# zwu88/TANTE

Measured on AMD Instinct MI355X. Metric: rollout frames/sec (fwd), TANTE on 256x256 Active Matter, higher is better.
Workload: dtype bf16

## Files before the change

### tante_amd/_lib.py

```python
import ctypes as C
import os

HERE = os.path.dirname(os.path.abspath(__file__))
LIB_PATH = os.environ.get("TANTE_LIB") or os.path.join(HERE, "lib", "libtante_hip.so")

F32, BF16 = 0, 1
ACT_NONE, ACT_GELU_ERF, ACT_GELU_TANH, ACT_RELU = 0, 1, 2, 3
A_LINEAR, A_PATCH_NHWC, A_PATCH_NCHW = 0, 1, 2
E_LINEAR, E_FILM, E_DECONV_NHWC, E_DECONV_NCHW = 0, 1, 2, 3
W_LINEAR, W_CONV_NHWC, W_DECONV_NHWC, W_DECONV_NCHW = 0, 1, 2, 3
W_LINEAR_T, W_CONV_NHWC_T, W_DECONV_NHWC_T, W_DECONV_NCHW_T = 4, 5, 6, 7

c_i32, c_i64, c_f32, c_vp = C.c_int32, C.c_int64, C.c_float, C.c_void_p


class PackGeom(C.Structure):
    _fields_ = [("n_pad", c_i32), ("k_pad", c_i32), ("nt", c_i32), ("cb", c_i32), ("bytes", c_i64)]


class Gemm(C.Structure):
    _fields_ = [
        ("a", c_vp), ("a_dtype", c_i32), ("a_mode", c_i32), ("M", c_i32), ("K", c_i32),
        ("a_s1", c_i64), ("a_s0", c_i64), ("a_off", c_i64), ("a_n0", c_i32),
        ("Hin", c_i32), ("Win", c_i32), ("Cin", c_i32), ("P", c_i32), ("ln", c_i32), ("ln_eps", c_f32),
# ... 144 lines not shown
                                   c_i64, c_i64, c_vp, c_vp], c_i32),
    "tante_cross_attention": ([c_vp, c_vp, c_vp, c_vp, c_i32, c_i64, c_i32, c_i32, c_i32, c_i32, c_i64, c_i64, c_i64, c_vp], c_i32),
    "tante_cvit_chain512": ([c_vp, c_vp, c_i64, c_vp, c_vp, c_vp, c_vp, c_f32, c_f32, c_f32, c_vp, c_vp, c_i32, c_i64, c_i32, c_vp, c_vp], c_i32),
    "tante_cvit_chain512_qkv": ([c_vp, c_vp, c_i64, c_vp, c_vp, c_f32, c_f32, c_i64, c_vp, c_vp, c_vp], c_i32),
    "tante_cross_attention_q": ([c_vp, c_vp, c_vp, c_vp, c_i32, c_i64, c_i32, c_i32, c_i32, c_i32, c_i64, c_i64, c_i64, c_i64, c_vp], c_i32),
    "tante_cross_attention_bwd": ([c_vp] * 9 + [c_i32, c_i64, c_i32, c_i32, c_i32, c_i32, c_i64, c_i64, c_i64, c_i64, c_vp], c_i32),
    "tante_layernorm_affine_bwd": ([c_vp, c_i32, c_vp, c_i32, c_vp, c_i64, c_i32, c_f32, c_vp, c_vp, c_vp, c_vp], c_i32),
    "tante_grid_embed_bwd": ([c_vp] * 5 + [c_i64, c_i32, c_i32, c_f32, c_vp, c_vp, c_vp, c_vp], c_i32),
    "tante_grid_embed": ([c_vp, c_vp, c_vp, c_i64, c_i32, c_i32, c_f32, c_vp, c_vp], c_i32),
    "tante_fourier_embed": ([c_vp, c_vp, c_i64, c_i32, c_vp, c_vp], c_i32),
    "tante_metric_sums": ([c_vp, c_i64, c_i64, c_i64, c_i64, c_vp, c_i32, c_i32, c_i64, c_i32, c_vp, c_vp], c_i32),
    "tante_mse_grad": ([c_vp, c_i64, c_i64, c_i64, c_i64, c_vp, c_i32, c_i32, c_i64, c_i32, c_f32, c_vp, c_vp], c_i32),
    "tante_sumsq": ([c_vp, c_i64, c_vp, c_vp], c_i32),
    "tante_adamw_step": ([c_vp, c_vp, c_vp, c_vp, c_i64, c_vp, c_f32, c_f32, c_f32, c_f32, c_f32, c_f32, c_i32, c_f32, c_vp], c_i32),
    "tante_layernorm_fwd": ([c_vp, c_i64, c_i32, c_f32, c_vp, c_i32, c_vp, c_vp], c_i32),
    "tante_layernorm_bwd": ([c_vp, c_i32, c_vp, c_vp, c_vp, c_i64, c_i32, c_vp, c_vp], c_i32),
    "tante_act_fwd": ([c_vp, c_i32, c_vp, c_i32, c_i64, c_i32, c_vp], c_i32),
    "tante_act_bwd": ([c_vp, c_i32, c_vp, c_i32, c_vp, c_i32, c_i64, c_i32, c_vp], c_i32),
    "tante_colsum": ([c_vp, c_i32, c_i64, c_i32, c_i64, c_vp, c_i32, c_vp], c_i32),
    "tante_film_pos_fwd": ([c_vp, c_vp, c_vp, c_vp, c_i64, c_i32, c_i32, c_i64, c_vp, c_vp], c_i32),
    "tante_pos_embed_tmajor": ([c_vp, c_vp, c_vp, c_i64, c_i32, c_i64, c_i32, c_vp, c_vp], c_i32),
    "tante_film_pos_bwd": ([c_vp, c_vp, c_vp, c_i64, c_i64, c_i32, c_i32, c_vp, c_vp, c_vp, c_vp, c_vp], c_i32),
    "tante_taylor_bwd": ([c_vp, c_i64, C.POINTER(c_vp), c_i32, C.c_double, c_i32, c_vp, c_i64, c_i32, c_i64, c_i64, c_vp], c_i32),
    "tante_attention_bwd": ([c_vp, c_vp, c_vp, c_i32, c_i32, c_i32, C.POINTER(Seq), c_i32, c_f32, C.c_uint64, c_vp], c_i32),
    "tante_attention_dropout": ([c_vp, c_vp, c_i32, c_i32, c_i32, C.POINTER(Seq), c_i32, c_f32, C.c_uint64, c_vp], c_i32),
    "tante_dropout_add": ([c_vp, c_i32, c_vp, c_f32, C.c_uint64, c_i64, c_vp, c_vp], c_i32),
    "tante_dropout_bwd": ([c_vp, c_f32, C.c_uint64, c_i64, c_vp, c_i32, c_vp], c_i32),
    "tante_axis_mlp_bwd": ([c_vp, c_vp, c_i64, c_i32, c_i64, c_vp, c_vp, c_vp, c_vp, c_vp, c_vp, c_vp], c_i32),
    "tante_fold_fwd": ([c_vp, c_vp, c_vp, c_vp, c_i32, c_i32, c_vp, c_vp, c_vp], c_i32),
    "tante_fold_bwd": ([c_vp, c_vp, c_vp, c_vp, c_vp, c_i32, c_i32, c_vp, c_vp, c_vp, c_vp, c_vp], c_i32),
    "tante_fold_bwd_clear": ([c_vp, c_vp, c_vp, c_vp, c_vp, c_i32, c_i32, c_vp, c_vp, c_vp, c_vp, c_vp], c_i32),
    "tante_fold_bwd_multi": ([c_vp, c_i32, c_i32, c_vp], c_i32),
    "tante_fold_fwd_multi": ([c_vp, c_i32, c_vp], c_i32),
    "tante_axis_mlp_film_supported": ([c_i64, c_i32, c_i32, c_i64, c_i32], c_i32),
    "tante_axis_mlp_film": ([c_vp, c_vp, c_vp, c_vp, c_vp, c_i64, c_i32, c_i32, c_i64, c_i32, c_vp, c_vp, c_vp, c_vp, c_vp], c_i32),
    "tante_film_pos_fwd_frames": ([c_vp, c_vp, c_vp, c_vp, c_i64, c_i32, c_i64, c_i32, c_vp, c_vp], c_i32),
    "tante_film_pos_bwd_frames": ([c_vp, c_vp, c_vp, c_i64, c_i64, c_i32, c_i32, c_vp, c_vp, c_vp, c_vp, c_vp], c_i32),
    "tante_film_pos_bwd_frames_acc": ([c_vp, c_vp, c_vp, c_i64, c_i64, c_i32, c_i32, c_vp, c_i32, c_vp, c_vp, c_vp, c_i32, c_vp], c_i32),
    "tante_film_table_bwd": ([c_vp, c_i32, c_i32] + [c_vp] * 6 + [c_vp, c_vp] + [c_vp] * 8 + [c_i32, c_vp], c_i32),
    "tante_pack_block_train_multi": ([c_vp, c_i32, c_i32, c_i32, c_vp], c_i32),
    "tante_pack_block_tail_bwd_multi": ([c_vp, c_i32, c_i32, c_i32, c_vp], c_i32),
    "tante_axis_mlp_bwd_fused_supported": ([c_i32, c_i64], c_i32),
    "tante_axis_mlp_bwd_fused": ([c_vp, c_vp, c_i64, c_i32, c_i64, c_vp, c_vp, c_vp, c_vp, c_vp, c_vp, c_vp, c_vp, c_vp], c_i32),
    "tante_axis_mlp_bwd_fused_ws": ([c_vp, c_vp, c_i64, c_i32, c_i64, c_vp, c_vp, c_vp, c_vp, c_vp, c_vp, c_vp, c_vp, c_vp, c_i64, c_vp], c_i32),
    "tante_axis_wgrad": ([c_vp, c_vp, c_i64, c_i32, c_i64, c_vp, c_vp, c_i32, c_vp], c_i32),
    "tante_axis_wgrad_workspace_bytes": ([], c_i64),
    "tante_set_seed_mix": ([c_vp], c_i32),
    "tante_axis_wgrad_ws": ([c_vp, c_vp, c_i64, c_i32, c_i64, c_vp, c_vp, c_i32, c_vp, c_i64, c_vp], c_i32),
    "tante_wgrad": ([C.POINTER(RowMat), C.POINTER(RowMat), c_i64, c_i32, c_i32, c_vp, c_vp, c_i32, c_i32, c_i32, c_i32, c_i32, c_i32, c_vp], c_i32),
    "tante_wgrad_ws": ([C.POINTER(RowMat), C.POINTER(RowMat), c_i64, c_i32, c_i32, c_vp, c_vp, c_i32, c_i32, c_i32, c_i32, c_i32, c_i32, c_vp, c_i64, c_vp], c_i32),
    "tante_wgrad_multi_ws": ([c_vp, c_vp, c_i32, c_i64, c_i32, c_i32, c_vp, c_vp, c_i32, c_i32, c_i32, c_i32, c_i32, c_i32, c_vp, c_i64, c_vp], c_i32),
    "tante_wgrad_multi": ([c_vp, c_vp, c_i32, c_i64, c_i32, c_i32, c_vp, c_vp, c_i32, c_i32, c_i32, c_i32, c_i32, c_i32, c_vp], c_i32),
    "tante_clip_value": ([c_vp, c_i64, c_f32, c_vp], c_i32),
    "tante_rt_reduce_bwd": ([c_vp, c_i32, c_i32, c_vp, c_vp], c_i32),
    "tante_last_error": ([], C.c_char_p),
    "tante_abi_version": ([], c_i32),
    "tante_set_option": ([C.c_char_p, c_i32], c_i32),
    "tante_nan_to_num": ([c_vp, c_vp, c_i64, c_vp], c_i32),
    "tante_head_fused_multi": ([c_i32, c_vp, c_vp, c_vp, c_i32, c_i64, c_i64, c_i64, c_i32, c_i32, c_i32, c_i32, c_i32, c_vp, c_i64, c_vp, c_i64,
                               c_vp], c_i32),
    "tante_head_fused_multi_streams": ([c_i32, c_vp, c_vp, c_vp, c_i32, c_i64, c_i64, c_i64, c_i32, c_i32, c_i32, c_i32, c_i32, c_vp, c_i64, c_vp, c_i64,
                               c_vp], c_i32),
    "tante_spectral_bf16out_supported": ([c_i64, c_i32, c_i32, c_i32, c_i32, c_i32, c_i32], c_i32),
    "tante_spectral_layer_bf16out": ([c_vp, c_i64, c_i32, c_i32, c_i32, c_vp, c_vp, c_i32, c_i32, c_i32, c_i32, c_vp, c_vp, c_i32, c_i32, c_vp, c_vp,
                                     c_i64, c_vp], c_i32),
    "tante_get_option": ([C.c_char_p, c_i32], c_i32),
    "tante_attention_masked": ([c_vp, c_vp, c_i32, c_i32, c_i32, c_i32, c_i32, c_i32, c_vp, c_i64, c_vp, c_vp], c_i32),
    "tante_attention_masked_bwd": ([c_vp, c_vp, c_vp, c_i32, c_i32, c_i32, c_i32, c_i32, c_i32, c_vp, c_i64, c_vp, c_vp, c_vp], c_i32),
    "tante_attention_flash_stats_floats": ([c_i32, C.POINTER(Seq)], c_i64),
    "tante_attention_flash_supported": ([c_i32, c_i32, c_i32, c_i32], c_i32),
    "tante_attention_flash": ([c_vp, c_vp, c_vp, c_i32, c_i32, c_i32, C.POINTER(Seq), c_i32, c_f32, C.c_uint64, c_vp], c_i32),
    "tante_attention_flash_bwd": ([c_vp, c_vp, c_vp, c_vp, c_vp, c_i32, c_i32, c_i32, C.POINTER(Seq), c_i32, c_f32, C.c_uint64, c_vp], c_i32),
    "tante_attention_flash_masked": ([c_vp, c_vp, c_vp, c_i32, c_i32, c_i32, c_i32, c_i32, c_i32, c_vp, c_i64, c_vp, c_f32, C.c_uint64, c_vp], c_i32),
    "tante_attention_flash_masked_bwd": ([c_vp, c_vp, c_vp, c_vp, c_vp, c_i32, c_i32, c_i32, c_i32, c_i32, c_i32, c_vp, c_i64, c_vp, c_f32, C.c_uint64, c_vp], c_i32),
    "tante_head_enc_supported": ([c_i32, c_i32], c_i32),
    "tante_head_enc_stream_bytes": ([c_i32], c_i64),
    "tante_head_enc_ws_bytes": ([c_i64], c_i64),
    "tante_pack_head_enc": ([c_vp] * 6 + [c_i32, c_i32, c_vp, c_vp], c_i32),
    "tante_head_enc_fused": ([c_i32, c_vp, c_vp, c_vp, c_i32, c_i64, c_i64, c_i64, c_i32, c_i32, c_i32, c_i32, c_i32, c_vp, c_i64, c_vp, c_i64,
                             c_vp, c_vp, c_vp, c_i64, c_vp], c_i32),
}

LIB_OPTIONS = ("TANTE_ATTN_BWD_HG", "TANTE_ATTN_BWD_NO_SPLIT", "TANTE_ATTN_BWD_VALU", "TANTE_ATTN_FWD_VALU", "TANTE_AXIS_BWD_SMALL_WGS",
               "TANTE_AXIS_BWD_WGS", "TANTE_AXIS_CT", "TANTE_AXIS_FILM", "TANTE_AXIS_GENERIC", "TANTE_AXIS_MFMA", "TANTE_AXIS_NT", "TANTE_AXIS_WGRAD_WGS",
               "TANTE_BLOCK_KERNEL", "TANTE_COLSUM_ROWS", "TANTE_CVIT_CHAIN_TOKENS", "TANTE_ENC23_SPLIT", "TANTE_FILM_BWD_ROWS",
               "TANTE_FS_GROUPS", "TANTE_FS_HALF", "TANTE_FS_SKEW", "TANTE_FS_WAVES", "TANTE_GEMM_NO_LITE", "TANTE_GEMM_SMALLM", "TANTE_GEMM_WGS", "TANTE_HEAD_WAVES",
               "TANTE_IM2COL_TILED", "TANTE_RESIZE_TILED", "TANTE_SPECTRAL_BF16OUT", "TANTE_SPECTRAL_DFT", "TANTE_SPECTRAL_X3", "TANTE_WGRAD_DEEP",
               "TANTE_WGRAD_JOBS", "TANTE_WGRAD_JOBS_WGS", "TANTE_WGRAD_NO_SLAB", "TANTE_WGRAD_NO_TR", "TANTE_WGRAD_REDUCE_NY",
               "TANTE_WGRAD_RG", "TANTE_WGRAD_SLAB_WGS", "TANTE_WGRAD_TR_WGS", "TANTE_WGRAD_WGS", "TANTE_XATTN_GPW", "TANTE_XATTN_VALU",)


_lib = None
ABI_VERSION = 14


def lib():
    global _lib
    if _lib is None:
        if not os.path.exists(LIB_PATH):
            raise RuntimeError(
                f"{LIB_PATH} is missing: build it with `python -m tante_amd.build` "
                "(or __graft_entry__.build()).  tante_amd has no CPU / eager fallback.")
        L = C.CDLL(LIB_PATH)
        for name, (argtypes, restype) in SIGNATURES.items():
            fn = getattr(L, name)
            fn.argtypes = argtypes
            fn.restype = restype
        got = int(L.tante_abi_version())
        if got != ABI_VERSION:
            raise RuntimeError(f"{LIB_PATH}: library ABI {got}, this binding expects {ABI_VERSION} -- a stale build (or a stale variant under "
                               "TANTE_LIB); rebuild with `python -m tante_amd.build`")
        _lib = L
        import warnings
        for k in LIB_OPTIONS:
            v = os.environ.get(k)
            if v is None:
                continue
            try:
                rc = L.tante_set_option(k.encode(), int(v))
            except ValueError:
                warnings.warn(f"{k}={v!r}: library options are integers; ignored")
                continue
            if rc != 0:
                warnings.warn(f"{k}={v}: tante_set_option refused it ({L.tante_last_error().decode(errors='replace')})")
    return _lib


def set_option(name: str, value: int) -> None:
    check(lib().tante_set_option(name.encode(), int(value)), "tante_set_option")


def get_option(name: str, default: int = 0) -> int:
    return int(lib().tante_get_option(name.encode(), int(default)))


def check(rc: int, what: str = ""):
    if rc != 0:
        msg = lib().tante_last_error().decode(errors="replace")
        raise RuntimeError(f"libtante_hip {what} failed (rc={rc}): {msg}")
```

### tante_amd/csrc/pointwise.hip

```cpp
#include "common.hip.h"
#include <stdlib.h>
#include <string.h>
#include <mutex>
#include <algorithm>

int tante_axis_mlp_mfma_supported(int64_t outer, int n, int64_t inner, const void* x, const void* w1, const void* w2);
int tante_axis_mlp_mfma(float* x, int64_t outer, int n, int64_t inner, const float* w1, const float* b1, const float* w2, const float* b2, hipStream_t s);

namespace {

template <int N>
__global__ __launch_bounds__(256) void axis_mlp_kernel(float* __restrict__ x, long outer, int n, long inner,
                                                       const float* __restrict__ w1, const float* __restrict__ b1,
                                                       const float* __restrict__ w2, const float* __restrict__ b2) {
  __shared__ __attribute__((aligned(16))) float w1s[N * N];
  __shared__ __attribute__((aligned(16))) float w2ts[N * N];
  __shared__ __attribute__((aligned(16))) float b1s[N];
  __shared__ __attribute__((aligned(16))) float b2s[N];
  for (int idx = threadIdx.x; idx < N * N; idx += 256) {
    const int j = idx / N, a = idx % N;
    const bool in = (j < n) && (a < n);
    w1s[idx] = in ? w1[j * n + a] : 0.0f;
    w2ts[idx] = in ? w2[a * n + j] : 0.0f;
  }
// ... 333 lines not shown
    const int tokn = i >> 2, q = i & 3, h = tokn / nW, w = tokn - h * nW;
    f32x4 v = *(const f32x4*)(lsrc + (long)tokn * C + q * 4);
    if (S.src) {
      const f32x4 a = *(const f32x4*)(fa + q * 4), b = *(const f32x4*)(fb + q * 4), sv = *(const f32x4*)(S.se + (long)tokn * C + c0 + q * 4);
      v = v * a + b + sv;
    }
    float2* d = (float2*)(plane + h * rs + w * AXWS + q * 4);
    d[0] = make_float2(v[0], v[1]);
    d[1] = make_float2(v[2], v[3]);
  }
  __syncthreads();
  if (!(dbg & 2)) axis_phase<BF16, MT>(plane, wst, wh1, bh1, wh2, bh2, nH, nW, rs, AXWS, tid);
  if (!(dbg & 4) && !(dbg & 1)) {
    axis_phase<BF16, MT>(plane, wst, ww1, bw1, ww2, bw2, nW, nH, AXWS, rs, tid, gx, (long)C, (long)nW * C);
    return;
  }
  if (!(dbg & 4)) axis_phase<BF16, MT>(plane, wst, ww1, bw1, ww2, bw2, nW, nH, AXWS, rs, tid);
  if (!(dbg & 1))
  for (int i = tid; i < nH * nW * 4; i += AXT) {
    const int tokn = i >> 2, q = i & 3, h = tokn / nW, w = tokn - h * nW;
    const float2* sp = (const float2*)(plane + h * rs + w * AXWS + q * 4);
    const float2 a = sp[0], b = sp[1];
    *(f32x4*)(gx + (long)tokn * C + q * 4) = f32x4{a.x, a.y, b.x, b.y};
  }
}

typedef __attribute__((ext_vector_type(2))) float f32x2;
__host__ __device__ constexpr int axe_rs(int nW, int ct) { return nW * ct + 32; }

template <int MT>
struct AxeW {
  static constexpr int KB = (MT + 1) / 2;
  u32x4 a1[MT][KB], a2[MT][KB];
  f32x4 b1[MT], b2[MT];
};

template <int MT>
__host__ __device__ constexpr int axe_wbytes() { return 2 * MT * ((MT + 1) / 2) * 1024 + 2 * 16 * MT * 4; }

template <int MT, int NT>
__device__ __forceinline__ void axe_stage_weights(const float* __restrict__ w1, const float* __restrict__ b1, const float* __restrict__ w2,
                                                  const float* __restrict__ b2, char* wst, int tid) {
  constexpr int N = 16 * MT, KB = (MT + 1) / 2;
  unsigned short* f = (unsigned short*)wst;
  for (int i = tid; i < N * N; i += NT) {
    const int row = i / N, col = i - row * N;
    const int mt = row >> 4, l15 = row & 15;
    {
      const int ks = col >> 5, e = (col & 31) >> 2, kk = col & 3;
      __bf16 v = (__bf16)w1[i];
      f[(mt * KB + ks) * 512 + (kk * 16 + l15) * 8 + e] = __builtin_bit_cast(unsigned short, v);
    }
    {
      const int tile = col >> 4, ks = tile >> 1, kk = (col & 15) >> 2, e = (tile & 1) * 4 + (col & 3);
      __bf16 v = (__bf16)w2[i];
      f[(MT * KB + mt * KB + ks) * 512 + (kk * 16 + l15) * 8 + e] = __builtin_bit_cast(unsigned short, v);
    }
  }
  float* bs = (float*)(wst + 2 * MT * KB * 1024);
  if (tid < N) { bs[tid] = b1[tid]; bs[N + tid] = b2[tid]; }
}

template <int MT>
__device__ __forceinline__ void axe_load_weights(const char* wst, int lane, int kk, AxeW<MT>& W) {
  constexpr int N = 16 * MT, KB = AxeW<MT>::KB;
  const u32x4* f = (const u32x4*)wst;
  const float* bs = (const float*)(wst + 2 * MT * KB * 1024);
#pragma unroll
  for (int mt = 0; mt < MT; ++mt) {
#pragma unroll
    for (int ks = 0; ks < KB; ++ks) {
      W.a1[mt][ks] = f[(mt * KB + ks) * 64 + lane];
      W.a2[mt][ks] = f[(MT * KB + mt * KB + ks) * 64 + lane];
      if (2 * ks + 1 >= MT) {
        W.a1[mt][ks][2] = W.a1[mt][ks][3] = 0u;
        W.a2[mt][ks][2] = W.a2[mt][ks][3] = 0u;
      }
    }
    W.b1[mt] = *(const f32x4*)(bs + mt * 16 + 4 * kk);
    W.b2[mt] = *(const f32x4*)(bs + N + mt * 16 + 4 * kk);
  }
}

template <int MT, int CT, int NWV, int NG, int LS, int GS, bool GOUT, int IL = 1>
__device__ __forceinline__ void axe_phase(float* plane, const AxeW<MT>& W, int wave, int l15, int kk, float* __restrict__ gout, long gls,
                                          long ggs) {
  constexpr int KB = AxeW<MT>::KB, NIT = CT == 32 ? NG : NG / 2, NE = 8 * KB;
  static_assert(CT == 32 || NG % 2 == 0, "16-channel tiles process line groups in pairs");
  const int gsel = CT == 32 ? 0 : (l15 >> 3), cp = CT == 32 ? 2 * l15 : 2 * (l15 & 7);
  constexpr int GPI = CT == 32 ? 1 : 2;
  auto gather = [&](int it, f32x2 (&xv)[NE]) {
    const float* base = plane + (GPI * it + gsel) * GS + cp + kk * LS;
#pragma unroll
    for (int ks = 0; ks < KB; ++ks)
#pragma unroll
      for (int e = 0; e < 8; ++e)
        if (ks * 32 + 4 * e < 16 * MT) xv[ks * 8 + e] = *(const f32x2*)(base + (ks * 32 + 4 * e) * LS);
        else xv[ks * 8 + e] = f32x2{0.f, 0.f};
  };
  f32x2 xa[IL][NE], xn[IL][NE];
#pragma unroll
  for (int g = 0; g < IL; ++g)
    if (wave + g * NWV < NIT) gather(wave + g * NWV, xa[g]);
  for (int it0 = wave; it0 < NIT; it0 += IL * NWV) {
#pragma unroll
    for (int g = 0; g < IL; ++g)
      if (it0 + (IL + g) * NWV < NIT) gather(it0 + (IL + g) * NWV, xn[g]);
    f32x4 out[IL][2][MT];
#pragma unroll
    for (int a = 0; a < 2; ++a) {
      u32x4 xb[IL][KB];
#pragma unroll
      for (int g = 0; g < IL; ++g)
#pragma unroll
        for (int ks = 0; ks < KB; ++ks)
#pragma unroll
          for (int q = 0; q < 4; ++q) xb[g][ks][q] = pack_bf16x2(xa[g][ks * 8 + 2 * q][a], xa[g][ks * 8 + 2 * q + 1][a]);
      f32x4 d1[IL][2 * KB];
#pragma unroll
      for (int g = 0; g < IL; ++g)
#pragma unroll
        for (int mt = 0; mt < 2 * KB; ++mt) d1[g][mt] = mt < MT ? W.b1[mt < MT ? mt : 0] : f32x4{0.f, 0.f, 0.f, 0.f};
#pragma unroll
      for (int mt = 0; mt < MT; ++mt)
#pragma unroll
        for (int ks = 0; ks < KB; ++ks)
#pragma unroll
          for (int g = 0; g < IL; ++g)
            d1[g][mt] = __builtin_amdgcn_mfma_f32_16x16x32_bf16(__builtin_bit_cast(bf16x8, W.a1[mt][ks]), __builtin_bit_cast(bf16x8, xb[g][ks]), d1[g][mt], 0, 0, 0);
#pragma unroll
      for (int g = 0; g < IL; ++g)
#pragma unroll
        for (int mt = 0; mt < MT; ++mt) d1[g][mt] = gelu_poly4<false>(d1[g][mt]);
      u32x4 hb[IL][KB];
#pragma unroll
      for (int g = 0; g < IL; ++g)
#pragma unroll
        for (int ks = 0; ks < KB; ++ks) {
          const f32x4 lo = d1[g][2 * ks], hi = d1[g][2 * ks + 1];
          hb[g][ks] = u32x4{pack_bf16x2(lo[0], lo[1]), pack_bf16x2(lo[2], lo[3]), pack_bf16x2(hi[0], hi[1]), pack_bf16x2(hi[2], hi[3])};
        }
#pragma unroll
      for (int mt = 0; mt < MT; ++mt) {
#pragma unroll
        for (int g = 0; g < IL; ++g) out[g][a][mt] = W.b2[mt];
#pragma unroll
        for (int ks = 0; ks < KB; ++ks)
#pragma unroll
          for (int g = 0; g < IL; ++g)
            out[g][a][mt] = __builtin_amdgcn_mfma_f32_16x16x32_bf16(__builtin_bit_cast(bf16x8, W.a2[mt][ks]), __builtin_bit_cast(bf16x8, hb[g][ks]), out[g][a][mt], 0, 0, 0);
      }
    }
#pragma unroll
    for (int g = 0; g < IL; ++g) {
      const int it = it0 + g * NWV;
      if (it < NIT) {
        float* rbase = plane + (GPI * it + gsel) * GS + cp + 4 * kk * LS;
        float* gbase = GOUT ? gout + (long)(GPI * it + gsel) * ggs + cp + 4 * kk * gls : nullptr;
#pragma unroll
        for (int mt = 0; mt < MT; ++mt)
#pragma unroll
          for (int r = 0; r < 4; ++r) {
            f32x2 v = *(const f32x2*)(rbase + (16 * mt + r) * LS);
            v[0] += out[g][0][mt][r];
            v[1] += out[g][1][mt][r];
#ifdef AXE_PLAIN_STORE
            if constexpr (GOUT) *(f32x2*)(gbase + (long)(16 * mt + r) * gls) = v;
#else
            if constexpr (GOUT) st_wt8(gbase + (long)(16 * mt + r) * gls, __builtin_bit_cast(u32x2, v));
#endif
            else *(f32x2*)(rbase + (16 * mt + r) * LS) = v;
          }
      }
    }
#pragma unroll
    for (int g = 0; g < IL; ++g)
#pragma unroll
      for (int j = 0; j < NE; ++j) xa[g][j] = xn[g][j];
  }
}

#ifdef TANTE_ABLATE
unsigned long long* g_axe_stamps = nullptr;
#define AXE_STAMP(k)                                                                  \
  do {                                                                                \
    if (stamps) {                                                                     \
      const unsigned long long t_ = __builtin_amdgcn_s_memtime();                     \
      if (lane == 0) stamps[((long)blockIdx.x * 16 + wave) * 12 + (k)] = t_;          \
    }                                                                                 \
  } while (0)
#else
#define AXE_STAMP(k)
#endif

template <int MTH, int MTW, int CT, int NT>
__global__ __launch_bounds__(NT) void axis_hw_exact_kernel(float* __restrict__ x, AxisSrc S, int C, const float* __restrict__ wh1,
                                                           const float* __restrict__ bh1, const float* __restrict__ wh2,
                                                           const float* __restrict__ bh2, const float* __restrict__ ww1,
                                                           const float* __restrict__ bw1, const float* __restrict__ ww2,
                                                           const float* __restrict__ bw2, unsigned long long* stamps,
                                                           const float* __restrict__ xin, float* __restrict__ xmid) {
  constexpr int NH = 16 * MTH, NW = 16 * MTW, RS = axe_rs(NW, CT), NWV = NT / 64;
  constexpr int AXE_IL = (NT == 512 && CT == 32 && MTH <= 2 && MTW <= 2) ? 2 : 1;
  constexpr int TPI = 256 / CT, LPT = CT / 4;
  extern __shared__ __attribute__((aligned(16))) float plane[];
  const int tid = threadIdx.x, lane = tid & 63, wave = tid >> 6, kk = lane >> 4, l15 = lane & 15;
  const int ctiles = C / CT;
  unsigned wg = blockIdx.x;
  if (gridDim.x % 8 == 0) wg = (blockIdx.x & 7) * (gridDim.x >> 3) + (blockIdx.x >> 3);
  const long bt = wg / ctiles;
  const int c0 = (wg % ctiles) * CT;
  float* gx = x + bt * (long)NH * NW * C + c0;
  AXE_STAMP(0);
#ifdef TANTE_ABLATE
  if (stamps && lane == 0) stamps[((long)blockIdx.x * 16 + wave) * 12 + 8] = __builtin_amdgcn_s_memrealtime();
#endif
  constexpr int IPR = NW / TPI;
  if (!S.src) {
    const float* gin = xin ? xin + (gx - x) : gx;
    for (int q = wave; q < NH * IPR; q += NWV) {
      const int h = q / IPR, j = q - h * IPR;
      const float* g = gin + ((long)h * NW + j * TPI + lane / LPT) * C + (lane % LPT) * 4;
      __builtin_amdgcn_global_load_lds((const __attribute__((address_space(1))) void*)g,
                                       (__attribute__((address_space(3))) void*)(plane + h * RS + j * 256), 16, 0, 0);
    }
  } else {
    const long b = bt / S.T, t = bt - b * S.T;
    const float* lsrc = S.src + t * S.t_stride + b * S.b_stride + c0;
    const int q4 = (lane % LPT) * 4;
    const f32x4 fa = *(const f32x4*)(S.fa + t * C + c0 + q4), fb = *(const f32x4*)(S.fb + t * C + c0 + q4);
    for (int q = wave; q < NH * IPR; q += NWV) {
      const int h = q / IPR, j = q - h * IPR, tokn = h * NW + j * TPI + lane / LPT;
      const f32x4 v = *(const f32x4*)(lsrc + (long)tokn * C + q4), sv = *(const f32x4*)(S.se + (long)tokn * C + c0 + q4);
      *(f32x4*)(plane + h * RS + j * 256 + lane * 4) = v * fa + fb + sv;
    }
  }
  char* wstH = (char*)(plane + NH * RS);
  char* wstW = wstH + axe_wbytes<MTH>();
  axe_stage_weights<MTH, NT>(wh1, bh1, wh2, bh2, wstH, tid);
  axe_stage_weights<MTW, NT>(ww1, bw1, ww2, bw2, wstW, tid);
  AXE_STAMP(1);
  __builtin_amdgcn_s_waitcnt(0x0070);
  AXE_STAMP(2);
  __syncthreads();
  AXE_STAMP(3);
  {
    AxeW<MTH> WH;
    axe_load_weights<MTH>(wstH, lane, kk, WH);
    axe_phase<MTH, CT, NWV, NW, RS, CT, false, AXE_IL>(plane, WH, wave, l15, kk, nullptr, 0, 0);
  }
  AXE_STAMP(4);
  AxeW<MTW> WW;
  axe_load_weights<MTW>(wstW, lane, kk, WW);
  __syncthreads();
  AXE_STAMP(5);
  if (xmid) {
    float* gm = xmid + (gx - x);
    for (int q = wave; q < NH * IPR; q += NWV) {
      const int h = q / IPR, j = q - h * IPR;
      *(f32x4*)(gm + ((long)h * NW + j * TPI + lane / LPT) * C + (lane % LPT) * 4) = *(const f32x4*)(plane + h * RS + j * 256 + lane * 4);
    }
  }
  axe_phase<MTW, CT, NWV, NH, CT, RS, true, AXE_IL>(plane, WW, wave, l15, kk, gx, (long)C, (long)NW * C);
  AXE_STAMP(6);
#ifdef TANTE_ABLATE
  if (stamps) {
    __builtin_amdgcn_s_waitcnt(0x0070);
    AXE_STAMP(7);
    if (lane == 0) stamps[((long)blockIdx.x * 16 + wave) * 12 + 9] = __builtin_amdgcn_s_memrealtime();
  }
#endif
}

__global__ void film_table_kernel(const float* __restrict__ t, int rows, int C, const float* __restrict__ sc_w0,
                                  const float* __restrict__ sc_b0, const float* __restrict__ sc_w2, const float* __restrict__ sc_b2,
                                  const float* __restrict__ sh_w0, const float* __restrict__ sh_b0, const float* __restrict__ sh_w2,
                                  const float* __restrict__ sh_b2, const float* __restrict__ add, float* __restrict__ a_out,
                                  float* __restrict__ b_out) {
  const int idx = blockIdx.x * blockDim.x + threadIdx.x;
  if (idx >= rows * C) return;
  const int r = idx / C, c = idx % C, Hd = C / 2;
  const float tv = t[r];
  float sa = sc_b2[c], sb = sh_b2[c];
  for (int j = 0; j < Hd; ++j) {
    sa += sc_w2[c * Hd + j] * fmaxf(sc_w0[j] * tv + sc_b0[j], 0.0f);
    sb += sh_w2[c * Hd + j] * fmaxf(sh_w0[j] * tv + sh_b0[j], 0.0f);
  }
  a_out[idx] = 1.0f + sa;
  b_out[idx] = sb + (add ? add[idx] : 0.0f);
}

__global__ __launch_bounds__(256) void film_table_bwd_kernel(const float* __restrict__ t, int rows, int C, const float* __restrict__ sc_w0,
                                                            const float* __restrict__ sc_b0, const float* __restrict__ sc_w2,
                                                            const float* __restrict__ sh_w0, const float* __restrict__ sh_b0,
                                                            const float* __restrict__ sh_w2, const float* __restrict__ dA,
                                                            const float* __restrict__ dB, float* g_sc_w0, float* g_sc_b0, float* g_sc_w2,
                                                            float* g_sc_b2, float* g_sh_w0, float* g_sh_b0, float* g_sh_w2, float* g_sh_b2,
                                                            int acc) {
  __shared__ float red[4][8][8];
  const int Hd = C / 2, tid = threadIdx.x, m = blockIdx.y, j0 = blockIdx.x * 8;
// ... 238 lines not shown
    hipLaunchKernelGGL(axis_mlp_lds_kernel, dim3((unsigned)((cols + 63) / 64)), dim3(64), lds, s, x, outer, n, inner, w1, b1, w2, b2);
  }
  TANTE_CHECK_LAUNCH();
  return 0;
}

template <bool BF16, int MT>
static void launch_axis_hw(float* x, const AxisSrc& S, long BT, int nH, int nW, int C, const float* wh1, const float* bh1, const float* wh2,
                           const float* bh2, const float* ww1, const float* bw1, const float* ww2, const float* bw2, size_t lds,
                           hipStream_t s) {
  static size_t attr = 0;
  if (lds > attr) {
    hipFuncSetAttribute((const void*)axis_hw_kernel<BF16, MT>, hipFuncAttributeMaxDynamicSharedMemorySize, (int)lds);
    attr = lds;
  }
  hipLaunchKernelGGL((axis_hw_kernel<BF16, MT>), dim3((unsigned)(BT * (C / 16))), dim3(AXT), lds, s, x, S, nH, nW, C, wh1, bh1, wh2, bh2,
                     ww1, bw1, ww2, bw2, tante_ablate_env("TANTE_AXIS_DEBUG"));
}

static int axis_hw_impl(float* x, const AxisSrc& S, int64_t BT, int nH, int nW, int C, const float* wh1, const float* bh1, const float* wh2,
                        const float* bh2, const float* ww1, const float* bw1, const float* ww2, const float* bw2, int compute, void* stream,
                        const float* xin = nullptr, float* xmid = nullptr);

#ifdef TANTE_ABLATE
extern "C" void tante_axe_set_stamps(unsigned long long* p) { g_axe_stamps = p; }
#endif

extern "C" int tante_axis_hw_train(const float* xin, float* xout, float* xmid, int64_t BT, int nH, int nW, int C, const float* wh1, const float* bh1,
                                   const float* wh2, const float* bh2, const float* ww1, const float* bw1, const float* ww2, const float* bw2,
                                   int compute, void* stream) {
  if (!xin || !xmid || ((uintptr_t)xin % 16) || ((uintptr_t)xmid % 16)) TANTE_FAIL(-1, "tante_axis_hw_train: null or misaligned pointer");
  const AxisSrc none = {nullptr, 0, 0, nullptr, nullptr, nullptr, 1};
  return axis_hw_impl(xout, none, BT, nH, nW, C, wh1, bh1, wh2, bh2, ww1, bw1, ww2, bw2, compute, stream, xin, xmid);
}

extern "C" int tante_axis_hw_oop(const float* xin, float* xout, int64_t BT, int nH, int nW, int C, const float* wh1, const float* bh1,
                                 const float* wh2, const float* bh2, const float* ww1, const float* bw1, const float* ww2, const float* bw2,
                                 int compute, void* stream) {
  if (!xin || ((uintptr_t)xin % 16) || xin == xout) TANTE_FAIL(-1, "tante_axis_hw_oop: null or misaligned source (or source == destination: use tante_axis_hw)");
  const AxisSrc none = {nullptr, 0, 0, nullptr, nullptr, nullptr, 1};
  return axis_hw_impl(xout, none, BT, nH, nW, C, wh1, bh1, wh2, bh2, ww1, bw1, ww2, bw2, compute, stream, xin, nullptr);
}

extern "C" int tante_axis_hw(float* x, int64_t BT, int nH, int nW, int C, const float* wh1, const float* bh1, const float* wh2,
                             const float* bh2, const float* ww1, const float* bw1, const float* ww2, const float* bw2,
                             int compute, void* stream) {
  const AxisSrc none = {nullptr, 0, 0, nullptr, nullptr, nullptr, 1};
  return axis_hw_impl(x, none, BT, nH, nW, C, wh1, bh1, wh2, bh2, ww1, bw1, ww2, bw2, compute, stream);
}

extern "C" int tante_axis_hw_film(float* x, const float* src, int64_t src_t_stride, int64_t src_b_stride, const float* film_a,
                                  const float* film_b, const float* s_emb, int T, int64_t BT, int nH, int nW, int C, const float* wh1,
                                  const float* bh1, const float* wh2, const float* bh2, const float* ww1, const float* bw1, const float* ww2,
                                  const float* bw2, int compute, void* stream) {
  if (!src || !film_a || !film_b || !s_emb || T <= 0 || BT % T) TANTE_FAIL(-1, "tante_axis_hw_film: bad argument");
  if (((uintptr_t)src | (uintptr_t)film_a | (uintptr_t)film_b | (uintptr_t)s_emb) % 16 || src_t_stride % 4 || src_b_stride % 4)
    TANTE_FAIL(-1, "tante_axis_hw_film: 16-byte alignment");
  const AxisSrc S = {src, (long)src_t_stride, (long)src_b_stride, film_a, film_b, s_emb, T};
  return axis_hw_impl(x, S, BT, nH, nW, C, wh1, bh1, wh2, bh2, ww1, bw1, ww2, bw2, compute, stream);
}

static int axis_hw_impl(float* x, const AxisSrc& S, int64_t BT, int nH, int nW, int C, const float* wh1, const float* bh1, const float* wh2,
                        const float* bh2, const float* ww1, const float* bw1, const float* ww2, const float* bw2, int compute, void* stream,
                        const float* xin, float* xmid) {
  if (!x || !wh1 || !bh1 || !wh2 || !bh2 || !ww1 || !bw1 || !ww2 || !bw2) TANTE_FAIL(-1, "tante_axis_hw: null pointer");
  if (BT <= 0 || nH <= 0 || nW <= 0 || C <= 0) TANTE_FAIL(-1, "tante_axis_hw: bad shape");
  hipStream_t s = (hipStream_t)stream;
  auto wbytes = [](int m) { return (size_t)(2 * m * ((m + 1) / 2) * 1024 + 2 * 16 * m * 4); };
  const size_t wst_bytes = wbytes(nH / 16) + wbytes(nW / 16);
  if (compute == TANTE_BF16 && nH % 16 == 0 && nW % 16 == 0 && nH <= 64 && nW <= 64 && C % 16 == 0 && ((uintptr_t)x % 16) == 0 &&
      (size_t)nH * axe_rs(nW, 16) * sizeof(float) + wst_bytes <= 160 * 1024 && !tante_opt("TANTE_AXIS_GENERIC", 0)) {
    const int force_ct = tante_opt("TANTE_AXIS_CT", 0);
    const bool fits32 = C % 32 == 0 && (size_t)nH * axe_rs(nW, 32) * sizeof(float) + wst_bytes <= 160 * 1024;
    const int ct = force_ct == 16 ? 16 : ((fits32 && (force_ct == 32 || BT * (C / 32) >= 192)) ? 32 : 16);
    const size_t elds = (size_t)nH * axe_rs(nW, ct) * sizeof(float) + wst_bytes;
    const unsigned grid = (unsigned)(BT * (C / ct));
    const int force_nt = tante_opt("TANTE_AXIS_NT", 0);
    const int nt32 = force_nt ? force_nt : ((nH <= 32 && nW <= 32) ? 1024 : 512);
#ifdef TANTE_ABLATE
    unsigned long long* axe_st = g_axe_stamps;
#else
    unsigned long long* axe_st = nullptr;
#endif
#define TANTE_AXE2(MH, MW, CTV, NTV)                                                                                                    \
  {                                                                                                                                     \
    static TantePerDevice attr;                                                                                                         \
    attr.once([&] { (void)hipFuncSetAttribute((const void*)axis_hw_exact_kernel<MH, MW, CTV, NTV>, hipFuncAttributeMaxDynamicSharedMemorySize, 160 * 1024); }); \
    hipLaunchKernelGGL((axis_hw_exact_kernel<MH, MW, CTV, NTV>), dim3(grid), dim3(NTV), elds, s, x, S, C, wh1, bh1, wh2, bh2, ww1, bw1, ww2, bw2, axe_st, xin, xmid); \
  }
#define TANTE_AXE(MH, MW)                  \
  {                                        \
    if (ct == 32 && nt32 == 1024) TANTE_AXE2(MH, MW, 32, 1024) \
    else if (ct == 32) TANTE_AXE2(MH, MW, 32, 512) \
    else TANTE_AXE2(MH, MW, 16, 512)       \
  }
    switch ((nH / 16) * 8 + nW / 16) {
      case 1 * 8 + 1: TANTE_AXE(1, 1); break; case 1 * 8 + 2: TANTE_AXE(1, 2); break; case 1 * 8 + 3: TANTE_AXE(1, 3); break; case 1 * 8 + 4: TANTE_AXE(1, 4); break;
      case 2 * 8 + 1: TANTE_AXE(2, 1); break; case 2 * 8 + 2: TANTE_AXE(2, 2); break; case 2 * 8 + 3: TANTE_AXE(2, 3); break; case 2 * 8 + 4: TANTE_AXE(2, 4); break;
      case 3 * 8 + 1: TANTE_AXE(3, 1); break; case 3 * 8 + 2: TANTE_AXE(3, 2); break; case 3 * 8 + 3: TANTE_AXE(3, 3); break;
      case 4 * 8 + 1: TANTE_AXE(4, 1); break; case 4 * 8 + 2: TANTE_AXE(4, 2); break;
      default: TANTE_FAIL(-2, "tante_axis_hw: no whole-tile variant for %d x %d", nH, nW);
    }
#undef TANTE_AXE
#undef TANTE_AXE2
    TANTE_CHECK_LAUNCH();
    return 0;
  }
  if (xin || xmid) TANTE_FAIL(-2, "tante_axis_hw_train: needs the whole-tile bf16 form (nH, nW multiples of 16, the plane within the LDS)");
  const int nmax = nH > nW ? nH : nW;
  const size_t lds = (((size_t)nH * axis_row_stride(nW) + 3) & ~(size_t)3) * sizeof(float) + 2 * (size_t)nmax * sizeof(float) +
                     2 * (size_t)nmax * (compute == TANTE_BF16 ? (nmax + 8) * 2 : nmax * 4);
  if (nmax > 64 || C % 16 || lds > 160 * 1024 || ((uintptr_t)x % 16))
    TANTE_FAIL(-2, "tante_axis_hw: needs nH, nW <= 64, C %% 16 == 0 and the plane to fit LDS (use tante_axis_mlp)");
  const int mt = (nmax + 15) / 16;
#define TANTE_AHW(BF, MTV) launch_axis_hw<BF, MTV>(x, S, (long)BT, nH, nW, C, wh1, bh1, wh2, bh2, ww1, bw1, ww2, bw2, lds, s)
  if (compute == TANTE_BF16) {
    switch (mt) { case 1: TANTE_AHW(true, 1); break; case 2: TANTE_AHW(true, 2); break; case 3: TANTE_AHW(true, 3); break; default: TANTE_AHW(true, 4); }
  } else {
    switch (mt) { case 1: TANTE_AHW(false, 1); break; case 2: TANTE_AHW(false, 2); break; case 3: TANTE_AHW(false, 3); break; default: TANTE_AHW(false, 4); }
  }
#undef TANTE_AHW
  TANTE_CHECK_LAUNCH();
  return 0;
}

extern "C" int tante_film_table(const float* t, int rows, int C, const float* sc_w0, const float* sc_b0, const float* sc_w2,
                                const float* sc_b2, const float* sh_w0, const float* sh_b0, const float* sh_w2,
                                const float* sh_b2, const float* add, float* a_out, float* b_out, void* stream) {
  if (!t || !sc_w0 || !sc_b0 || !sc_w2 || !sc_b2 || !sh_w0 || !sh_b0 || !sh_w2 || !sh_b2 || !a_out || !b_out)
    TANTE_FAIL(-1, "tante_film_table: null pointer");
  if (rows <= 0 || C <= 0 || C % 2) TANTE_FAIL(-1, "tante_film_table: bad shape");
  hipLaunchKernelGGL(film_table_kernel, dim3((rows * C + 255) / 256), dim3(256), 0, (hipStream_t)stream, t, rows, C, sc_w0, sc_b0,
                     sc_w2, sc_b2, sh_w0, sh_b0, sh_w2, sh_b2, add, a_out, b_out);
  TANTE_CHECK_LAUNCH();
  return 0;
}

extern "C" int tante_film_table_bwd(const float* t, int rows, int C, const float* sc_w0, const float* sc_b0, const float* sc_w2, const float* sh_w0,
                                    const float* sh_b0, const float* sh_w2, const float* dA, const float* dB, float* g_sc_w0, float* g_sc_b0,
                                    float* g_sc_w2, float* g_sc_b2, float* g_sh_w0, float* g_sh_b0, float* g_sh_w2, float* g_sh_b2,
                                    int accumulate, void* stream) {
  if (!t || !sc_w0 || !sc_b0 || !sc_w2 || !sh_w0 || !sh_b0 || !sh_w2 || !dA || !dB || !g_sc_w0 || !g_sc_b0 || !g_sc_w2 || !g_sc_b2 || !g_sh_w0 ||
      !g_sh_b0 || !g_sh_w2 || !g_sh_b2)
    TANTE_FAIL(-1, "tante_film_table_bwd: null pointer");
  if (rows <= 0 || rows > 8 || C <= 0 || C % 16) TANTE_FAIL(-2, "tante_film_table_bwd: rows <= 8 and C %% 16 == 0 expected (got %d x %d)", rows, C);
  hipLaunchKernelGGL(film_table_bwd_kernel, dim3((unsigned)(C / 16), 2), dim3(256), 0, (hipStream_t)stream, t, rows, C, sc_w0, sc_b0, sc_w2, sh_w0,
                     sh_b0, sh_w2, dA, dB, g_sc_w0, g_sc_b0, g_sc_w2, g_sc_b2, g_sh_w0, g_sh_b0, g_sh_w2, g_sh_b2, accumulate);
  TANTE_CHECK_LAUNCH();
  return 0;
}

extern "C" int tante_film_apply(const float* x, int64_t x_bstride, float* y, int64_t rows, int C, int64_t rows_per,
                                const float* a, const float* b, void* stream) {
  if (!x || !y || !a || !b) TANTE_FAIL(-1, "tante_film_apply: null pointer");
  if (rows <= 0 || C <= 0 || C % 4 || rows_per <= 0 || x_bstride % 4)
    TANTE_FAIL(-1, "tante_film_apply: bad shape (C and the batch stride must be multiples of 4)");
  const long n4 = rows * (C / 4);
  hipLaunchKernelGGL(film_apply_kernel, dim3((unsigned)((n4 + 255) / 256)), dim3(256), 0, (hipStream_t)stream, x,
                     (long)x_bstride, y, (long)rows, C / 4, (long)rows_per, a, b);
  TANTE_CHECK_LAUNCH();
  return 0;
}

extern "C" int tante_gather_last(const float* z, int64_t n, int E, float* out, void* stream) {
  if (!z || !out || n <= 0 || E <= 0) TANTE_FAIL(-1, "tante_gather_last: bad argument");
  hipLaunchKernelGGL(gather_last_kernel, dim3((unsigned)((n + 255) / 256)), dim3(256), 0, (hipStream_t)stream, z, (long)n, E, out);
  TANTE_CHECK_LAUNCH();
  return 0;
}

extern "C" int tante_format_input(const float* x, int64_t n_img, int T, int64_t HW, int D, float* out, int64_t out_bstride, void* stream) {
// ... 95 lines not shown
```

Before: 19040.

## Split axis-MLP plane load into column blocks overlapped with compute

```diff
diff --git a/tante_amd/_lib.py b/tante_amd/_lib.py
--- a/tante_amd/_lib.py
+++ b/tante_amd/_lib.py
@@ -250,7 +250,7 @@
 }
 
 LIB_OPTIONS = ("TANTE_ATTN_BWD_HG", "TANTE_ATTN_BWD_NO_SPLIT", "TANTE_ATTN_BWD_VALU", "TANTE_ATTN_FWD_VALU", "TANTE_AXIS_BWD_SMALL_WGS",
-               "TANTE_AXIS_BWD_WGS", "TANTE_AXIS_CT", "TANTE_AXIS_FILM", "TANTE_AXIS_GENERIC", "TANTE_AXIS_MFMA", "TANTE_AXIS_NT", "TANTE_AXIS_WGRAD_WGS",
+               "TANTE_AXIS_BLOCKS", "TANTE_AXIS_BWD_WGS", "TANTE_AXIS_CT", "TANTE_AXIS_FILM", "TANTE_AXIS_GENERIC", "TANTE_AXIS_MFMA", "TANTE_AXIS_NT", "TANTE_AXIS_WGRAD_WGS",
                "TANTE_BLOCK_KERNEL", "TANTE_COLSUM_ROWS", "TANTE_CVIT_CHAIN_TOKENS", "TANTE_ENC23_SPLIT", "TANTE_FILM_BWD_ROWS",
                "TANTE_FS_GROUPS", "TANTE_FS_HALF", "TANTE_FS_SKEW", "TANTE_FS_WAVES", "TANTE_GEMM_NO_LITE", "TANTE_GEMM_SMALLM", "TANTE_GEMM_WGS", "TANTE_HEAD_WAVES",
                "TANTE_IM2COL_TILED", "TANTE_RESIZE_TILED", "TANTE_SPECTRAL_BF16OUT", "TANTE_SPECTRAL_DFT", "TANTE_SPECTRAL_X3", "TANTE_WGRAD_DEEP",
diff --git a/tante_amd/csrc/pointwise.hip b/tante_amd/csrc/pointwise.hip
--- a/tante_amd/csrc/pointwise.hip
+++ b/tante_amd/csrc/pointwise.hip
@@ -439,11 +439,12 @@
   }
 }
 
-template <int MT, int CT, int NWV, int NG, int LS, int GS, bool GOUT, int IL = 1>
+template <int MT, int CT, int NWV, int NG, int LS, int GS, bool GOUT, int IL = 1, int IT0 = 0, int ITN = -1>
 __device__ __forceinline__ void axe_phase(float* plane, const AxeW<MT>& W, int wave, int l15, int kk, float* __restrict__ gout, long gls,
                                           long ggs) {
-  constexpr int KB = AxeW<MT>::KB, NIT = CT == 32 ? NG : NG / 2, NE = 8 * KB;
+  constexpr int KB = AxeW<MT>::KB, NIT = ITN < 0 ? (CT == 32 ? NG : NG / 2) : IT0 + ITN, NE = 8 * KB;
   static_assert(CT == 32 || NG % 2 == 0, "16-channel tiles process line groups in pairs");
+  static_assert(IT0 >= 0 && NIT <= (CT == 32 ? NG : NG / 2), "iteration range outside the phase");
   const int gsel = CT == 32 ? 0 : (l15 >> 3), cp = CT == 32 ? 2 * l15 : 2 * (l15 & 7);
   constexpr int GPI = CT == 32 ? 1 : 2;
   auto gather = [&](int it, f32x2 (&xv)[NE]) {
@@ -458,8 +459,8 @@
   f32x2 xa[IL][NE], xn[IL][NE];
 #pragma unroll
   for (int g = 0; g < IL; ++g)
-    if (wave + g * NWV < NIT) gather(wave + g * NWV, xa[g]);
-  for (int it0 = wave; it0 < NIT; it0 += IL * NWV) {
+    if (IT0 + wave + g * NWV < NIT) gather(IT0 + wave + g * NWV, xa[g]);
+  for (int it0 = IT0 + wave; it0 < NIT; it0 += IL * NWV) {
 #pragma unroll
     for (int g = 0; g < IL; ++g)
       if (it0 + (IL + g) * NWV < NIT) gather(it0 + (IL + g) * NWV, xn[g]);
@@ -550,7 +551,21 @@
 #define AXE_STAMP(k)
 #endif
 
-template <int MTH, int MTW, int CT, int NT>
+__host__ __device__ constexpr int axe_vmcnt(int n) {
+  return (n & 15) | ((n >> 4) << 14) | 0x0070 | 0x0F00;
+}
+__device__ __forceinline__ void axe_lds_barrier() { asm volatile("s_waitcnt lgkmcnt(0)\n\ts_barrier" ::: "memory"); }
+__host__ __device__ constexpr int axe_raw_floats(int nH, int nW) { return 2 * nH * nH + 2 * nW * nW + 4 * 64; }
+__host__ __device__ constexpr int axe_blocks(int mth, int mtw, int ct, int nt) {
+  const int nwv = nt / 64, ipr = 16 * mtw / (256 / ct), nith = ct == 32 ? 16 * mtw : 8 * mtw;
+  const int il = (nt == 512 && ct == 32 && mth <= 2 && mtw <= 2) ? 2 : 1;
+  const int nwi = (2 * 256 * mth * mth + 2 * 256 * mtw * mtw) / 256 + 4;
+  if (ipr % 2 || (16 * mth * (ipr / 2)) % nwv || (nith / 2) % (il * nwv)) return 0;
+  if ((nwi + nwv - 1) / nwv + 16 * mth * ipr / nwv > 63) return 0;
+  return 2;
+}
+
+template <int MTH, int MTW, int CT, int NT, int NB = 0>
 __global__ __launch_bounds__(NT) void axis_hw_exact_kernel(float* __restrict__ x, AxisSrc S, int C, const float* __restrict__ wh1,
                                                            const float* __restrict__ bh1, const float* __restrict__ wh2,
                                                            const float* __restrict__ bh2, const float* __restrict__ ww1,
@@ -573,6 +588,74 @@
   if (stamps && lane == 0) stamps[((long)blockIdx.x * 16 + wave) * 12 + 8] = __builtin_amdgcn_s_memrealtime();
 #endif
   constexpr int IPR = NW / TPI;
+  if constexpr (NB > 0) {
+    static_assert(NB == 2 && axe_blocks(MTH, MTW, CT, NT) == NB, "no column-block form for this variant");
+    constexpr int JPB = IPR / NB, DPW = NH * JPB / NWV;
+    constexpr int NITH = CT == 32 ? NW : NW / 2, GPB = NITH / NB;
+    constexpr int IH = NH * NH / 256, IW = NW * NW / 256, NWI = 2 * IH + 2 * IW + 4;
+    static_assert((NWI + NWV - 1) / NWV + NB * DPW <= 63, "the wave's outstanding DMA instructions must fit the 6-bit vmcnt counter");
+    char* wstH = (char*)(plane + NH * RS);
+    char* wstW = wstH + axe_wbytes<MTH>();
+    float* raw = (float*)(wstW + axe_wbytes<MTW>());
+    float* rawb = raw + 2 * NH * NH + 2 * NW * NW;
+    for (int i = wave; i < NWI; i += NWV) {
+      if (i < 2 * IH + 2 * IW) {
+        const float* w = i < IH ? wh1 : i < 2 * IH ? wh2 : i < 2 * IH + IW ? ww1 : ww2;
+        const int k = i < IH ? i : i < 2 * IH ? i - IH : i < 2 * IH + IW ? i - 2 * IH : i - 2 * IH - IW;
+        float* d = i < IH ? raw : i < 2 * IH ? raw + NH * NH : i < 2 * IH + IW ? raw + 2 * NH * NH : raw + 2 * NH * NH + NW * NW;
+        __builtin_amdgcn_global_load_lds((const __attribute__((address_space(1))) void*)(w + k * 256 + lane * 4),
+                                         (__attribute__((address_space(3))) void*)(d + k * 256), 16, 0, 0);
+      } else {
+        const int v = i - (2 * IH + 2 * IW), n = v < 2 ? NH : NW;
+        const float* bp = v == 0 ? bh1 : v == 1 ? bh2 : v == 2 ? bw1 : bw2;
+        __builtin_amdgcn_global_load_lds((const __attribute__((address_space(1))) void*)(bp + (lane < n ? lane : 0)),
+                                         (__attribute__((address_space(3))) void*)(rawb + v * 64), 4, 0, 0);
+      }
+    }
+    const float* gin = xin ? xin + (gx - x) : gx;
+    auto issue_block = [&](int b) {
+      for (int r = wave; r < NH * JPB; r += NWV) {
+        const int h = r / JPB, j = b * JPB + (r - h * JPB);
+        const float* g = gin + ((long)h * NW + j * TPI + lane / LPT) * C + (lane % LPT) * 4;
+        __builtin_amdgcn_global_load_lds((const __attribute__((address_space(1))) void*)g,
+                                         (__attribute__((address_space(3))) void*)(plane + h * RS + j * 256), 16, 0, 0);
+      }
+    };
+    issue_block(0);
+    AXE_STAMP(1);
+    __builtin_amdgcn_s_waitcnt(axe_vmcnt(DPW));
+    axe_lds_barrier();
+    axe_stage_weights<MTH, NT>(raw, rawb, raw + NH * NH, rawb + 64, wstH, tid);
+    axe_stage_weights<MTW, NT>(raw + 2 * NH * NH, rawb + 128, raw + 2 * NH * NH + NW * NW, rawb + 192, wstW, tid);
+    AXE_STAMP(2);
+    __builtin_amdgcn_s_waitcnt(axe_vmcnt(0));
+    axe_lds_barrier();
+    issue_block(1);
+    AXE_STAMP(3);
+    AxeW<MTH> WH;
+    axe_load_weights<MTH>(wstH, lane, kk, WH);
+    axe_phase<MTH, CT, NWV, NW, RS, CT, false, AXE_IL, 0, GPB>(plane, WH, wave, l15, kk, nullptr, 0, 0);
+    AXE_STAMP(10);
+    __builtin_amdgcn_s_waitcnt(axe_vmcnt(0));
+    axe_lds_barrier();
+    AXE_STAMP(11);
+    axe_phase<MTH, CT, NWV, NW, RS, CT, false, AXE_IL, GPB, GPB>(plane, WH, wave, l15, kk, nullptr, 0, 0);
+    AXE_STAMP(4);
+    AxeW<MTW> WW;
+    axe_load_weights<MTW>(wstW, lane, kk, WW);
+    __syncthreads();
+    AXE_STAMP(5);
+    axe_phase<MTW, CT, NWV, NH, CT, RS, true, AXE_IL>(plane, WW, wave, l15, kk, gx, (long)C, (long)NW * C);
+    AXE_STAMP(6);
+#ifdef TANTE_ABLATE
+    if (stamps) {
+      __builtin_amdgcn_s_waitcnt(0x0070);
+      AXE_STAMP(7);
+      if (lane == 0) stamps[((long)blockIdx.x * 16 + wave) * 12 + 9] = __builtin_amdgcn_s_memrealtime();
+    }
+#endif
+    return;
+  }
   if (!S.src) {
     const float* gin = xin ? xin + (gx - x) : gx;
     for (int q = wave; q < NH * IPR; q += NWV) {
@@ -977,11 +1060,26 @@
 #else
     unsigned long long* axe_st = nullptr;
 #endif
+    const size_t raw_bytes = (size_t)axe_raw_floats(nH, nW) * sizeof(float);
+    const bool blocks = tante_opt("TANTE_AXIS_BLOCKS", -1) != 0 && !S.src && !xmid && elds + raw_bytes <= 160 * 1024 &&
+                        (((uintptr_t)wh1 | (uintptr_t)wh2 | (uintptr_t)ww1 | (uintptr_t)ww2 | (uintptr_t)xin) % 16) == 0 && C % 4 == 0;
 #define TANTE_AXE2(MH, MW, CTV, NTV)                                                                                                    \
   {                                                                                                                                     \
-    static TantePerDevice attr;                                                                                                         \
-    attr.once([&] { (void)hipFuncSetAttribute((const void*)axis_hw_exact_kernel<MH, MW, CTV, NTV>, hipFuncAttributeMaxDynamicSharedMemorySize, 160 * 1024); }); \
-    hipLaunchKernelGGL((axis_hw_exact_kernel<MH, MW, CTV, NTV>), dim3(grid), dim3(NTV), elds, s, x, S, C, wh1, bh1, wh2, bh2, ww1, bw1, ww2, bw2, axe_st, xin, xmid); \
+    constexpr int NBV = axe_blocks(MH, MW, CTV, NTV);                                                                                   \
+    bool done = false;                                                                                                                  \
+    if constexpr (NBV > 0) {                                                                                                            \
+      if (blocks) {                                                                                                                     \
+        static TantePerDevice attrb;                                                                                                    \
+        attrb.once([&] { (void)hipFuncSetAttribute((const void*)axis_hw_exact_kernel<MH, MW, CTV, NTV, NBV>, hipFuncAttributeMaxDynamicSharedMemorySize, 160 * 1024); }); \
+        hipLaunchKernelGGL((axis_hw_exact_kernel<MH, MW, CTV, NTV, NBV>), dim3(grid), dim3(NTV), elds + raw_bytes, s, x, S, C, wh1, bh1, wh2, bh2, ww1, bw1, ww2, bw2, axe_st, xin, xmid); \
+        done = true;                                                                                                                    \
+      }                                                                                                                                 \
+    }                                                                                                                                   \
+    if (!done) {                                                                                                                        \
+      static TantePerDevice attr;                                                                                                       \
+      attr.once([&] { (void)hipFuncSetAttribute((const void*)axis_hw_exact_kernel<MH, MW, CTV, NTV>, hipFuncAttributeMaxDynamicSharedMemorySize, 160 * 1024); }); \
+      hipLaunchKernelGGL((axis_hw_exact_kernel<MH, MW, CTV, NTV>), dim3(grid), dim3(NTV), elds, s, x, S, C, wh1, bh1, wh2, bh2, ww1, bw1, ww2, bw2, axe_st, xin, xmid); \
+    }                                                                                                                                   \
   }
 #define TANTE_AXE(MH, MW)                  \
   {                                        \
```

New measurement: 19240 (median of 6 runs). +1.0%, better.
